# fchchen/omni-recall-rag

Measured on AMD Instinct MI355X. Metric: queries/sec at top-k=10 over N x 3072-d chunks; score delta vs C# reference in `parity`, higher is better.
Workload: dtype i8 screen + f32*f32->f64 exact re-score; 1 GPU; C3: 10000000 chunks x 3072-d fp32 on one GPU, batch=256 queries per step, top-k=10, full hybrid (cosine+keyword+recency), candidate_limit=corpus; corpus_rows=10000000

## Files before the change

### omni-recall-rag_amd/csrc/orr_epilogue.h

```cpp
#pragma once

#include "orr_kernels.h"
#include "orr_device.h"

#include <type_traits>

#include "orr_screen_tile16_asm.inc"

namespace orr {

typedef float f32x16 __attribute__((ext_vector_type(16)));
typedef __bf16 bf16x8 __attribute__((ext_vector_type(8)));
typedef __bf16 bf16x4 __attribute__((ext_vector_type(4)));
typedef int i32x16 __attribute__((ext_vector_type(16)));
typedef int i32x4e __attribute__((ext_vector_type(4)));

constexpr int kEpiQueue = 8;
struct EpiParked { float a; uint32_t idx; };

template <int NI, int NJ>
struct EpiTileLoads {
    double2 rc[NJ];
    float4 rf[NJ];
    uint32_t w[NI][NJ][kCountPlanes];
};

template <int NI, int NJ>
__device__ __forceinline__ void epilogue_issue_loads(EpiTileLoads<NI, NJ> &L, int qbase, int64_t colbase, int32_t B, int64_t n_rows,
                                                     const FusedEpilogue &epi, int lane)
{
    const int fr = lane & 31;
    const int32_t n_qg = (B + 31) >> 5;
    const bool has_rf = epi.i8_rowf != nullptr, has_cp = epi.count_planes != nullptr;
    const float4 *rowf = has_rf ? epi.i8_rowf : reinterpret_cast<const float4 *>(epi.rowc);
#pragma unroll
    for (int j = 0; j < NJ; ++j) {
        const int64_t col = colbase + j * 32 + fr;
        const uint32_t colc = (uint32_t)(col < n_rows ? col : n_rows - 1);
        L.rc[j] = load_global(epi.rowc, colc);
        const float4 rf = load_global(rowf, colc);
        L.rf[j] = has_rf ? rf : make_float4(1.f, 0.f, 0.f, 0.f);
#pragma unroll
        for (int i = 0; i < NI; ++i) {
            const int qg = (qbase + i * 32) >> 5;
            const int qgc = qg < n_qg ? qg : n_qg - 1;
#pragma unroll
            for (int p = 0; p < kCountPlanes; ++p) {
                const gptr<uint32_t> plane = as_global(has_cp ? epi.count_planes + ((int64_t)p * n_qg + qgc) * epi.plane_stride
                                                              : reinterpret_cast<const uint32_t *>(epi.rowc));
                const uint32_t wv = plane[colc];
                L.w[i][j][p] = has_cp ? wv : 0u;
            }
        }
    }
}

template <bool AGPR, typename T>
__device__ __forceinline__ float acc_as_float(T v)
{
    if constexpr (AGPR) {
        T r;
        asm("v_accvgpr_read_b32 %0, %1" : "=v"(r) : "a"(v));
        return (float)r;
    } else {
        return (float)v;
    }
}

struct EpiNoHook { __device__ __forceinline__ void operator()(int) const {} };

template <int NI, int NJ, bool RESCORED, typename ACC = f32x16, bool STAGED = false, int QDEPTH = kEpiQueue, bool AGPR = false,
          typename HOOK = EpiNoHook>
__device__ __forceinline__ void fused_epilogue(const ACC (&acc)[NI][NJ], int qbase, int64_t colbase, int32_t B,
                                               int64_t n_rows, const FusedEpilogue &epi, int lane, EpiParked *queue,
                                               int queue_stride, uint32_t idx_salt = 0, unsigned long long *st = nullptr,
                                               const EpiTileLoads<NI, NJ> *pre = nullptr, const float4 *qf_lds = nullptr,
                                               HOOK between_blocks = HOOK())
{
    constexpr bool INT_ACC = !__is_same(ACC, f32x16);
#define ORR_EPI_STAMP(k) if (st && lane == 0) st[k] = __builtin_amdgcn_s_memtime()
    const int fr = lane & 31, fh = lane >> 5;
    EpiTileLoads<NI, NJ> own;
    if constexpr (!STAGED) epilogue_issue_loads(own, qbase, colbase, B, n_rows, epi, lane);
    const EpiTileLoads<NI, NJ> &L = STAGED ? *pre : own;
    float rb[NJ], cj[NJ], eb[NJ];
    int64_t cols[NJ];
    bool ok[NJ];
#pragma unroll
    for (int j = 0; j < NJ; ++j) {
        cols[j] = colbase + j * 32 + fr;
        ok[j] = cols[j] < n_rows;
        rb[j] = (float)L.rc[j].x;
        const float rr = ok[j] ? (float)L.rc[j].y : -__builtin_huge_valf();
        float ea = 0.f;
        eb[j] = 0.f;
        if (epi.i8_rowf) {
            rb[j] *= L.rf[j].x;
            ea = L.rf[j].y; eb[j] = L.rf[j].z;
        }
        cj[j] = rr + ea;
    }
    if (st) { asm volatile("" :: "v"(cj[0]), "v"(rb[0]), "v"(eb[0])); ORR_EPI_STAMP(4); }
    int parked = 0;
    auto qf_of = [&](int i, int e) -> float4 {
        const int qi = qbase + i * 32 + (e & 3) + 8 * (e >> 2) + 4 * fh;
        if constexpr (STAGED) return qf_lds[i * 32 + (e & 3) + 8 * (e >> 2) + 4 * fh];
        else return epi.qf[qi < B ? qi : B - 1];
    };
#pragma unroll
    for (int i = 0; i < NI; ++i) {
        between_blocks(i);
        uint32_t w[NJ][kCountPlanes];
#pragma unroll
        for (int j = 0; j < NJ; ++j)
#pragma unroll
            for (int p = 0; p < kCountPlanes; ++p) w[j][p] = L.w[i][j][p] >> (16 * fh);
        const int q_left = B - (qbase + i * 32 + 4 * fh);
        if constexpr (STAGED) {
            unsigned long long wave_any = 0ull;
            float4 qfg[2][4];
#pragma unroll
            for (int e = 0; e < 4; ++e) qfg[0][e] = qf_of(i, e);
#pragma unroll
            for (int e0 = 0; e0 < 16; e0 += 4) {
                if (e0 + 4 < 16) {
#pragma unroll
                    for (int e = 0; e < 4; ++e) qfg[((e0 >> 2) + 1) & 1][e] = qf_of(i, e0 + 4 + e);
                }
                __builtin_amdgcn_sched_barrier(0);
                unsigned long long hit[4][NJ];
#pragma unroll
                for (int e1 = 0; e1 < 4; ++e1) {
                    const int e = e0 + e1;
                    const float4 qf = qfg[(e0 >> 2) & 1][e1];
#pragma unroll
                    for (int j = 0; j < NJ; ++j) {
                        const uint32_t m = (w[j][e >> 2] >> (4 * (e & 3))) & 15u;
                        const float a = acc_as_float<AGPR>(acc[i][j][e]);
                        const float upper = __builtin_fmaf((float)m, qf.z, __builtin_fmaf(a, qf.x * rb[j], __builtin_fmaf(qf.w, eb[j], cj[j])));
                        hit[e1][j] = __builtin_amdgcn_ballot_w64(!(upper < qf.y));
                    }
                }
#pragma unroll
                for (int e1 = 0; e1 < 4; ++e1)
#pragma unroll
                    for (int j = 0; j < NJ; ++j) wave_any |= hit[e1][j];
            }
            if (wave_any == 0ull) {
                if (i == 0) { ORR_EPI_STAMP(5); }
                continue;
            }
        }
#pragma unroll
        for (int e = 0; e < 16; ++e) {
            const int cb = (e & 3) + 8 * (e >> 2);
            const int qi = qbase + i * 32 + cb + 4 * fh;
            const float4 qf = qf_of(i, e);
            const bool has_query = cb < q_left;
#pragma unroll
            for (int j = 0; j < NJ; ++j) {
                const uint32_t m = (w[j][e >> 2] >> (4 * (e & 3))) & 15u;
                const float a = acc_as_float<AGPR>(acc[i][j][e]);
                const float upper = __builtin_fmaf((float)m, qf.z, __builtin_fmaf(a, qf.x * rb[j], __builtin_fmaf(qf.w, eb[j], cj[j])));
                bool drop = upper < qf.y;
                if constexpr (!INT_ACC) drop = drop && __builtin_fabsf(a) <= 3.4028234663852886e38f;
                drop = drop || !has_query || !ok[j];
                if (!drop) {
                    if (parked < QDEPTH) {
                        EpiParked pk;
                        pk.a = a; pk.idx = (uint32_t)((i * 16 + e) * NJ + j) + idx_salt;
                        queue[parked * queue_stride] = pk;
                    } else if (RESCORED) {
                        const uint32_t slot = atomicAdd(&epi.cnt[qi], 1u);
                        if (slot < epi.cap) {
                            SelEntry en;
                            en.key = ~0ull; en.pos = (uint32_t)cols[j]; en.pad = 0;
                            epi.buf[(int64_t)qi * epi.cap + slot] = en;
                        }
                    } else {
                        atomicAdd(&epi.cnt[qi], epi.cap + 1u);
                    }
                    ++parked;
                }
            }
        }
        if (i == 0) { ORR_EPI_STAMP(5); }
    }
    ORR_EPI_STAMP(6);
#undef ORR_EPI_STAMP
    if (parked > QDEPTH) parked = QDEPTH;
    for (int s = 0; s < parked; ++s) {
        EpiParked pk = queue[s * queue_stride];
        pk.idx -= idx_salt;
        const int j = (int)(pk.idx % NJ), ie = (int)(pk.idx / NJ), e = ie & 15, i = ie >> 4;
        const int qi = qbase + i * 32 + (e & 3) + 8 * (e >> 2) + 4 * fh;
        const int64_t col = colbase + j * 32 + fr;
        const QueryConst qc = epi.qc[qi];
        const double2 rc = epi.rowc[col];
        const uint32_t mm = qc.n_terms > 0 ? kw_matches(epi.kw, qi, (uint32_t)col) : 0u;
        double dot = (double)pk.a, bound = 0.0;
        if (epi.i8_rowf) {
            const float4 rf = epi.i8_rowf[col];
            dot *= (double)rf.x * (double)epi.i8_qs1[qi];
            bound = (double)rf.y + (double)epi.qf[qi].w * (double)rf.z;
        }
        unsigned long long key = score_key(fused_score_fast(dot, rc.x, rc.y, mm, qc) + bound);
        if (!(__builtin_fabsf(pk.a) <= 3.4028234663852886e38f) || !(bound <= 1.7976931348623157e308)) key = ~0ull;
        if (key > epi.tau[qi]) {
            const uint32_t slot = atomicAdd(&epi.cnt[qi], 1u);
            if (slot < epi.cap) {
                SelEntry en;
                en.key = key; en.pos = (uint32_t)col; en.pad = 0;
                epi.buf[(int64_t)qi * epi.cap + slot] = en;
            }
        }
    }
}

__device__ __forceinline__ int tile16_row(int m) { return (((0 - (m >> 2)) & 3) << 2) | (m & 3); }
__device__ __forceinline__ int tile16_c_of(int lane) { return tile16_row(lane & 15); }
__device__ __forceinline__ int tile16_g_of(int lane) { return (0 - (lane >> 4)) & 3; }

struct EpiTileLoads16 {
    double2 rc[8];
    float4 rf[8];
    uint32_t w[4][8][2];
};

template <int BITS = 4>
__device__ __forceinline__ void epilogue_word_offsets16(uint32_t (&at)[8], int64_t colbase, int32_t B, int64_t n_rows, const FusedEpilogue &epi,
                                                        int lane)
{
    const int c = tile16_c_of(lane), g = tile16_g_of(lane);
    const int32_t n_qg = (B + 31) >> 5;
    const uint32_t plane_dist = epi.count_planes && BITS == 4 ? (uint32_t)((int64_t)n_qg * epi.plane_stride) : 0u;
    const uint32_t col0 = (uint32_t)colbase + (uint32_t)c, last = (uint32_t)(n_rows - 1), half = (uint32_t)(g >> 1) * plane_dist;
#pragma unroll
    for (int j = 0; j < 8; ++j) {
        const uint32_t col = col0 + 16u * j;
        at[j] = (col < last ? col : last) + half;
    }
}

template <int BITS = 4>
__device__ __forceinline__ void epilogue_load_words16(uint32_t (&w)[8][2], const uint32_t (&at)[8], int b, int qbase, int32_t B,
                                                      const FusedEpilogue &epi)
{
    const int32_t n_qg = (B + 31) >> 5;
    const bool has_cp = epi.count_planes != nullptr;
    const int qg = (qbase >> 5) + b;
    const int qgc = qg < n_qg ? qg : n_qg - 1;
#pragma unroll
    for (int t = 0; t < 2; ++t) {
        const uint32_t *plane = has_cp ? epi.count_planes + ((int64_t)(BITS == 2 ? t : 2 * t) * n_qg + qgc) * epi.plane_stride
                                       : reinterpret_cast<const uint32_t *>(epi.rowc);
#pragma unroll
        for (int j = 0; j < 8; ++j) {
            const uint32_t wv = load_global_at<uint32_t>(plane, at[j] * 4u);
            w[j][t] = has_cp ? wv : 0u;
        }
    }
}

template <int BITS = 4>
__device__ __forceinline__ void epilogue_issue_loads16(EpiTileLoads16 &L, int qbase, int64_t colbase, int32_t B, int64_t n_rows,
                                                       const FusedEpilogue &epi, int lane)
{
    const uint32_t col0 = (uint32_t)colbase + (uint32_t)tile16_c_of(lane), last = (uint32_t)(n_rows - 1);
#pragma unroll
    for (int j = 0; j < 8; ++j) {
        const uint32_t col = col0 + 16u * j;
        const uint32_t off = (col < last ? col : last) * 16u;
        L.rc[j] = load_global_at_d2(epi.rowc, off);
        L.rf[j] = load_global_at_f4(epi.i8_rowf, off);
    }
    uint32_t at[8];
    epilogue_word_offsets16<BITS>(at, colbase, B, n_rows, epi, lane);
    epilogue_load_words16<BITS>(L.w[0], at, 0, qbase, B, epi);
}

template <int BITS = 4>
__device__ __forceinline__ void epilogue_issue_later_words16(EpiTileLoads16 &L, int qbase, int64_t colbase, int32_t B, int64_t n_rows,
                                                             const FusedEpilogue &epi, int lane)
{
    uint32_t at[8];
    epilogue_word_offsets16<BITS>(at, colbase, B, n_rows, epi, lane);
#pragma unroll
    for (int b = 1; b < 4; ++b) epilogue_load_words16<BITS>(L.w[b], at, b, qbase, B, epi);
}

template <int N, typename F>
__device__ __forceinline__ void static_for(F &&f)
{
    if constexpr (N > 0) {
        static_for<N - 1>(f);
        f(std::integral_constant<int, N - 1>{});
    }
}

template <int IDX>
__device__ __forceinline__ float acc16_as_float(int token)
{
    int r;
    asm("v_accvgpr_read_b32 %0, a[%1]" : "=v"(r) : "n"(IDX), "v"(token) : ORR_T16_ACC_CLOBBERS);
    return (float)r;
}

template <int IDX>
__device__ __forceinline__ float acc16_as_float_here(int token)
{
    int r;
    asm volatile("v_accvgpr_read_b32 %0, a[%1]" : "=v"(r) : "n"(IDX), "v"(token) : ORR_T16_ACC_CLOBBERS);
    return (float)r;
}

template <int IDX>
__device__ __forceinline__ int acc16_as_int_here(int token)
{
    int r;
    asm volatile("v_accvgpr_read_b32 %0, a[%1]" : "=v"(r) : "n"(IDX), "v"(token) : ORR_T16_ACC_CLOBBERS);
    return r;
}

typedef float f32x2e __attribute__((ext_vector_type(2)));

__host__ __device__ constexpr uint32_t count_nibbles_even(uint32_t w) { return w & 0x0F0F0F0Fu; }
__host__ __device__ constexpr uint32_t count_nibbles_odd(uint32_t w) { return (w >> 4) & 0x0F0F0F0Fu; }
__host__ __device__ constexpr uint32_t count_nibble_operand(int e, uint32_t x, uint32_t y) { return (e & 1) ? y : x; }
__host__ __device__ constexpr int count_nibble_byte(int e) { return e >> 1; }

__host__ __device__ constexpr uint32_t spread_count_fields2(uint32_t v)
{
    const uint32_t t = v | (v << 6);
    return (t | (t << 12)) & 0x03030303u;
}

namespace count_word_checks {
constexpr bool two_bit_spread_exact()
{
    for (uint32_t v = 0; v < 256u; ++v)
        for (int e = 0; e < 4; ++e)
            if (((spread_count_fields2(v) >> (8 * e)) & 0xFFu) != ((v >> (2 * e)) & 3u)) return false;
    return true;
}
constexpr bool nibble_extraction_exact()
{
    for (int h = 0; h < 2; ++h)
        for (int e = 0; e < 4; ++e)
            for (uint32_t v = 0; v < 16u; ++v)
                for (uint32_t bg : {0u, ~0u}) {
                    const int at = 16 * h + 4 * e;
                    const uint32_t w = (bg & ~(15u << at)) | (v << at);
                    const uint32_t half = w >> (16 * h);
                    const uint32_t op = count_nibble_operand(e, count_nibbles_even(half), count_nibbles_odd(half));
                    if (((op >> (8 * count_nibble_byte(e))) & 0xFFu) != v) return false;
                }
    return true;
}
}
static_assert(count_word_checks::two_bit_spread_exact(), "two-bit count words: field e of a byte must land in byte e");
static_assert(count_word_checks::nibble_extraction_exact(), "four-bit count words: nibble e must be byte (e >> 1) of x or y");

template <int E>
__device__ __forceinline__ float count_of_nibble(uint32_t x, uint32_t y)
{
    const uint32_t v = count_nibble_operand(E, x, y);
    float r;
    if constexpr (count_nibble_byte(E) == 0) asm("v_cvt_f32_ubyte0 %0, %1" : "=v"(r) : "v"(v));
    else asm("v_cvt_f32_ubyte1 %0, %1" : "=v"(r) : "v"(v));
    return r;
}

template <int BYTE>
__device__ __forceinline__ float ubyte_as_float(uint32_t v)
{
    float r;
    if constexpr (BYTE == 0) asm("v_cvt_f32_ubyte0 %0, %1" : "=v"(r) : "v"(v));
    else if constexpr (BYTE == 1) asm("v_cvt_f32_ubyte1 %0, %1" : "=v"(r) : "v"(v));
    else if constexpr (BYTE == 2) asm("v_cvt_f32_ubyte2 %0, %1" : "=v"(r) : "v"(v));
    else asm("v_cvt_f32_ubyte3 %0, %1" : "=v"(r) : "v"(v));
    return r;
}

template <int QDEPTH, typename HOOK = EpiNoHook, int BITS = 4>
__device__ __forceinline__ void fused_epilogue16(int acc_token, int qbase, int64_t colbase, int32_t B, int64_t n_rows,
                                                 const FusedEpilogue &epi, int lane, EpiParked *queue, int queue_stride, uint32_t idx_salt,
                                                 unsigned long long *st, const EpiTileLoads16 &L, const float4 *qf_lds,
                                                 HOOK between_blocks = HOOK())
{
#define ORR_EPI_STAMP(k) if (st && lane == 0) st[k] = __builtin_amdgcn_s_memtime()
    const int c = tile16_c_of(lane), g = tile16_g_of(lane);
    const int sh = 16 * (g & 1);
    const float qw_max = qf_lds[0].w;
    f32x2e rb2[4], cjw2[4];
    const int64_t col0 = colbase + c;
#pragma unroll
    for (int j = 0; j < 8; ++j) {
        const float rbv = (float)L.rc[j].x * L.rf[j].x;
        const float cj = (float)L.rc[j].y + L.rf[j].y, eb = L.rf[j].z;
        const bool keep_all = !(rbv <= 1e30f) || !(eb <= 1e30f) || !(cj <= 3.0e38f) || !(cj >= -3.0e38f);
        const float cjw = keep_all ? __builtin_huge_valf() : __builtin_fmaf(qw_max, eb, cj);
        rb2[j >> 1][j & 1] = keep_all ? 0.f : rbv;
        cjw2[j >> 1][j & 1] = col0 + j * 16 < n_rows ? cjw : -__builtin_huge_valf();
    }
    if (st) { asm volatile("" :: "v"(cjw2[0][0]), "v"(rb2[0][0])); ORR_EPI_STAMP(4); }
    int parked = 0;
    const float4 *qf_lane = qf_lds + 4 * g;
    uint32_t group_flags = 0u;
    static_for<4>([&](auto b_c) {
        constexpr int b = decltype(b_c)::value;
        between_blocks(b);
        static_for<2>([&](auto t_c) {
            constexpr int t = decltype(t_c)::value;
            f32x2e qx2[4], qz2[4], nqy2[4];
            float mx[4];
#pragma unroll
            for (int e = 0; e < 4; ++e) {
                const float4 qf = qf_lane[32 * b + 16 * t + e];
                qx2[e] = f32x2e{qf.x, qf.x}; qz2[e] = f32x2e{qf.z, qf.z}; nqy2[e] = f32x2e{-qf.y, -qf.y};
                mx[e] = -__builtin_huge_valf();
            }
            static_for<4>([&](auto jp_c) {
                constexpr int jp = decltype(jp_c)::value, j0 = 2 * jp;
                uint32_t x0, y0, x1, y1;
                if constexpr (BITS == 2) {
                    x0 = spread_count_fields2(__builtin_amdgcn_ubfe(L.w[b][j0][t], 8u * (uint32_t)g, 8u));
                    x1 = spread_count_fields2(__builtin_amdgcn_ubfe(L.w[b][j0 + 1][t], 8u * (uint32_t)g, 8u));
                    y0 = y1 = 0u;
                } else {
                    const uint32_t w0 = L.w[b][j0][t] >> sh, w1 = L.w[b][j0 + 1][t] >> sh;
                    x0 = count_nibbles_even(w0); y0 = count_nibbles_odd(w0); x1 = count_nibbles_even(w1); y1 = count_nibbles_odd(w1);
                }
                static_for<4>([&](auto e_c) {
                    constexpr int e = decltype(e_c)::value;
                    const f32x2e a2 = {acc16_as_float<4 * (8 * (2 * b + t) + j0) + e>(acc_token), acc16_as_float<4 * (8 * (2 * b + t) + j0 + 1) + e>(acc_token)};
                    f32x2e m2;
                    if constexpr (BITS == 2) m2 = f32x2e{ubyte_as_float<e>(x0), ubyte_as_float<e>(x1)};
                    else m2 = f32x2e{count_of_nibble<e>(x0, y0), count_of_nibble<e>(x1, y1)};
                    const f32x2e t1 = a2 * rb2[jp];
                    const f32x2e t2 = __builtin_elementwise_fma(t1, qx2[e], cjw2[jp]);
                    const f32x2e t3 = __builtin_elementwise_fma(m2, qz2[e], t2);
                    const f32x2e d = t3 + nqy2[e];
                    mx[e] = __builtin_fmaxf(__builtin_fmaxf(mx[e], d[0]), d[1]);
                });
            });
#pragma unroll
            for (int e = 0; e < 4; ++e) {
                const unsigned long long group_any = __builtin_amdgcn_ballot_w64(mx[e] >= 0.f);
                group_flags |= group_any != 0ull ? 1u << (8 * b + 4 * t + e) : 0u;
            }
            asm volatile("" :: "s"(group_flags));
        });
        if constexpr (b == 0) { ORR_EPI_STAMP(5); }
    });
    int token_1b = acc_token;
    asm volatile("" : "+v"(token_1b));
    static_for<4>([&](auto b_c) {
        constexpr int b = decltype(b_c)::value;
        if (((group_flags >> (8 * b)) & 0xffu) != 0u) {
            uint32_t at1[8], w1[8][2];
            epilogue_word_offsets16<BITS>(at1, colbase, B, n_rows, epi, lane);
            epilogue_load_words16<BITS>(w1, at1, b, qbase, B, epi);
            static_for<8>([&](auto te_c) {
                constexpr int te = decltype(te_c)::value, t = te >> 2, e = te & 3, i = 2 * b + t;
                if ((group_flags & (1u << (8 * b + te))) == 0u) return;
                const int qi = qbase + 16 * i + 4 * g + e;
                const float4 q1 = qf_lane[32 * b + 16 * t + e];
                const bool has_query = qi < B;
                static_for<8>([&](auto j_c) {
                    constexpr int j = decltype(j_c)::value;
                    const uint32_t m = BITS == 2 ? (w1[j][t] >> (8 * g + 2 * e)) & 3u : ((w1[j][t] >> sh) >> (4 * e)) & 15u;
                    const float a = acc16_as_float_here<4 * (8 * i + j) + e>(token_1b);
                    const float upper = __builtin_fmaf((float)m, q1.z, __builtin_fmaf(a * rb2[j >> 1][j & 1], q1.x, cjw2[j >> 1][j & 1]));
                    const bool drop = upper < q1.y || !has_query || !(col0 + j * 16 < n_rows);
                    if (!drop) {
                        if (parked < QDEPTH) {
                            EpiParked pk;
                            pk.a = a; pk.idx = (uint32_t)((i * 4 + e) * 8 + j) + idx_salt;
                            queue[parked * queue_stride] = pk;
                        } else {
                            const uint32_t slot = atomicAdd(&epi.cnt[qi], 1u);
                            if (slot < epi.cap) {
                                SelEntry en;
                                en.key = ~0ull; en.pos = (uint32_t)(col0 + j * 16); en.pad = 0;
                                epi.buf[(int64_t)qi * epi.cap + slot] = en;
                            }
                        }
                        ++parked;
                    }
                });
            });
        }
    });
    ORR_EPI_STAMP(6);
#undef ORR_EPI_STAMP
    if (parked > QDEPTH) parked = QDEPTH;
    for (int s = 0; s < parked; ++s) {
        EpiParked pk = queue[s * queue_stride];
        pk.idx -= idx_salt;
        const int j = (int)(pk.idx & 7u), ie = (int)(pk.idx >> 3), e = ie & 3, i = ie >> 2;
        const int qi = qbase + 16 * i + 4 * g + e;
        const int64_t col = colbase + j * 16 + c;
        const QueryConst qc = epi.qc[qi];
        const double2 rc = epi.rowc[col];
        const uint32_t mm = qc.n_terms > 0 ? kw_matches(epi.kw, qi, (uint32_t)col) : 0u;
        const float4 rf = epi.i8_rowf[col];
        const double dot = (double)pk.a * ((double)rf.x * (double)epi.i8_qs1[qi]);
        const double bound = (double)rf.y + (double)epi.qf[qi].w * (double)rf.z;
        unsigned long long key = score_key(fused_score_fast(dot, rc.x, rc.y, mm, qc) + bound);
        if (!(bound <= 1.7976931348623157e308)) key = ~0ull;
        if (key > epi.tau[qi]) {
            const uint32_t slot = atomicAdd(&epi.cnt[qi], 1u);
            if (slot < epi.cap) {
                SelEntry en;
                en.key = key; en.pos = (uint32_t)col; en.pad = 0;
                epi.buf[(int64_t)qi * epi.cap + slot] = en;
            }
        }
    }
}

}
```

Before: 31390 queries/s.

## Add coarse per-lane bound gate before per-column screen bound evaluation

Replaces the per-column float bound computation in the screening epilogue with a two-level gate. First, each lane takes the max integer accumulator over its 8 columns, combined with the max row scale, the max offset and an OR/max-combined keyword count field, to form a cheap upper bound per query group. Only groups whose coarse bound passes run the finer per-column float bound, which now uses the group-wide count bound instead of per-column counts. This cuts VALU work and count-field unpacking in the common all-rejected case. In exchange, the finer pass is looser on the count term, so slightly more groups may reach the exact stage, and it adds a second accumulator-read pass for the groups that pass.

```diff
diff --git a/omni-recall-rag_amd/csrc/orr_epilogue.h b/omni-recall-rag_amd/csrc/orr_epilogue.h
--- a/omni-recall-rag_amd/csrc/orr_epilogue.h
+++ b/omni-recall-rag_amd/csrc/orr_epilogue.h
@@ -307,6 +307,14 @@
 }
 
 template <int IDX>
+__device__ __forceinline__ int acc16_as_int(int token)
+{
+    int r;
+    asm("v_accvgpr_read_b32 %0, a[%1]" : "=v"(r) : "n"(IDX), "v"(token) : ORR_T16_ACC_CLOBBERS);
+    return r;
+}
+
+template <int IDX>
 __device__ __forceinline__ float acc16_as_float_here(int token)
 {
     int r;
@@ -324,63 +332,50 @@
 
 typedef float f32x2e __attribute__((ext_vector_type(2)));
 
-__host__ __device__ constexpr uint32_t count_nibbles_even(uint32_t w) { return w & 0x0F0F0F0Fu; }
-__host__ __device__ constexpr uint32_t count_nibbles_odd(uint32_t w) { return (w >> 4) & 0x0F0F0F0Fu; }
-__host__ __device__ constexpr uint32_t count_nibble_operand(int e, uint32_t x, uint32_t y) { return (e & 1) ? y : x; }
-__host__ __device__ constexpr int count_nibble_byte(int e) { return e >> 1; }
-
-__host__ __device__ constexpr uint32_t spread_count_fields2(uint32_t v)
-{
-    const uint32_t t = v | (v << 6);
-    return (t | (t << 12)) & 0x03030303u;
-}
+template <int BITS, int N>
+__host__ __device__ constexpr uint32_t count_group_bound(const uint32_t (&w)[N])
+{
+    uint32_t any = 0u, three = 0u;
+    for (int j = 0; j < N; ++j) {
+        any |= w[j];
+        if (BITS == 2) three |= w[j] & (w[j] >> 1);
+    }
+    return BITS == 2 ? any & ~(any & (any >> 1) & ~three & 0x55555555u) : any;
+}
+template <int BITS>
+__host__ __device__ constexpr uint32_t count_lane_fields(uint32_t w, int g) { return BITS == 2 ? w >> (8 * g) : w >> (16 * (g & 1)); }
+template <int BITS>
+__host__ __device__ constexpr uint32_t count_field_of(uint32_t lane_fields, int e) { return (lane_fields >> (BITS * e)) & ((1u << BITS) - 1u); }
 
 namespace count_word_checks {
-constexpr bool two_bit_spread_exact()
-{
-    for (uint32_t v = 0; v < 256u; ++v)
-        for (int e = 0; e < 4; ++e)
-            if (((spread_count_fields2(v) >> (8 * e)) & 0xFFu) != ((v >> (2 * e)) & 3u)) return false;
+template <int BITS, int ROWS>
+constexpr bool group_bound_covers_every_row()
+{
+    constexpr uint32_t top = (1u << BITS) - 1u;
+    uint32_t combos = 1u;
+    for (int r = 0; r < ROWS; ++r) combos *= top + 1u;
+    for (int g = 0; g < 4; ++g)
+        for (int e = 0; e < 4; ++e) {
+            const int at = BITS == 2 ? 8 * g + 2 * e : 16 * (g & 1) + 4 * e;
+            for (uint32_t c = 0; c < combos; ++c)
+                for (uint32_t bg : {0u, ~0u}) {
+                    uint32_t w[ROWS] = {}, largest = 0u, ored = 0u;
+                    for (uint32_t r = 0, rest = c; r < (uint32_t)ROWS; ++r, rest >>= BITS) {
+                        const uint32_t v = rest & top;
+                        w[r] = ((r & 1u ? ~bg : bg) & ~(top << at)) | (v << at);
+                        largest = v > largest ? v : largest;
+                        ored |= v;
+                        if (count_field_of<BITS>(count_lane_fields<BITS>(w[r], g), e) != v) return false;
+                    }
+                    const uint32_t got = count_field_of<BITS>(count_lane_fields<BITS>(count_group_bound<BITS>(w), g), e);
+                    if (BITS == 2 ? got != largest : (got != ored || got < largest)) return false;
+                }
+        }
     return true;
 }
-constexpr bool nibble_extraction_exact()
-{
-    for (int h = 0; h < 2; ++h)
-        for (int e = 0; e < 4; ++e)
-            for (uint32_t v = 0; v < 16u; ++v)
-                for (uint32_t bg : {0u, ~0u}) {
-                    const int at = 16 * h + 4 * e;
-                    const uint32_t w = (bg & ~(15u << at)) | (v << at);
-                    const uint32_t half = w >> (16 * h);
-                    const uint32_t op = count_nibble_operand(e, count_nibbles_even(half), count_nibbles_odd(half));
-                    if (((op >> (8 * count_nibble_byte(e))) & 0xFFu) != v) return false;
-                }
-    return true;
-}
-}
-static_assert(count_word_checks::two_bit_spread_exact(), "two-bit count words: field e of a byte must land in byte e");
-static_assert(count_word_checks::nibble_extraction_exact(), "four-bit count words: nibble e must be byte (e >> 1) of x or y");
-
-template <int E>
-__device__ __forceinline__ float count_of_nibble(uint32_t x, uint32_t y)
-{
-    const uint32_t v = count_nibble_operand(E, x, y);
-    float r;
-    if constexpr (count_nibble_byte(E) == 0) asm("v_cvt_f32_ubyte0 %0, %1" : "=v"(r) : "v"(v));
-    else asm("v_cvt_f32_ubyte1 %0, %1" : "=v"(r) : "v"(v));
-    return r;
-}
-
-template <int BYTE>
-__device__ __forceinline__ float ubyte_as_float(uint32_t v)
-{
-    float r;
-    if constexpr (BYTE == 0) asm("v_cvt_f32_ubyte0 %0, %1" : "=v"(r) : "v"(v));
-    else if constexpr (BYTE == 1) asm("v_cvt_f32_ubyte1 %0, %1" : "=v"(r) : "v"(v));
-    else if constexpr (BYTE == 2) asm("v_cvt_f32_ubyte2 %0, %1" : "=v"(r) : "v"(v));
-    else asm("v_cvt_f32_ubyte3 %0, %1" : "=v"(r) : "v"(v));
-    return r;
-}
+}
+static_assert(count_word_checks::group_bound_covers_every_row<2, 3>(), "two-bit count words: a field of the group's word must be the largest of the rows' fields");
+static_assert(count_word_checks::group_bound_covers_every_row<4, 2>(), "four-bit count words: a field of the group's word must be >= that field of every row");
 
 template <int QDEPTH, typename HOOK = EpiNoHook, int BITS = 4>
 __device__ __forceinline__ void fused_epilogue16(int acc_token, int qbase, int64_t colbase, int32_t B, int64_t n_rows,
@@ -398,63 +393,74 @@
     for (int j = 0; j < 8; ++j) {
         const float rbv = (float)L.rc[j].x * L.rf[j].x;
         const float cj = (float)L.rc[j].y + L.rf[j].y, eb = L.rf[j].z;
-        const bool keep_all = !(rbv <= 1e30f) || !(eb <= 1e30f) || !(cj <= 3.0e38f) || !(cj >= -3.0e38f);
+        const bool keep_all = !(rbv >= 0.f) || !(rbv <= 1e30f) || !(eb <= 1e30f) || !(cj <= 3.0e38f) || !(cj >= -3.0e38f);
         const float cjw = keep_all ? __builtin_huge_valf() : __builtin_fmaf(qw_max, eb, cj);
         rb2[j >> 1][j & 1] = keep_all ? 0.f : rbv;
         cjw2[j >> 1][j & 1] = col0 + j * 16 < n_rows ? cjw : -__builtin_huge_valf();
     }
     if (st) { asm volatile("" :: "v"(cjw2[0][0]), "v"(rb2[0][0])); ORR_EPI_STAMP(4); }
+    const float rb_max = __builtin_fmaxf(__builtin_fmaxf(__builtin_fmaxf(rb2[0][0], rb2[0][1]), __builtin_fmaxf(rb2[1][0], rb2[1][1])),
+                                         __builtin_fmaxf(__builtin_fmaxf(rb2[2][0], rb2[2][1]), __builtin_fmaxf(rb2[3][0], rb2[3][1])));
+    const float cjw_max = __builtin_fmaxf(__builtin_fmaxf(__builtin_fmaxf(cjw2[0][0], cjw2[0][1]), __builtin_fmaxf(cjw2[1][0], cjw2[1][1])),
+                                          __builtin_fmaxf(__builtin_fmaxf(cjw2[2][0], cjw2[2][1]), __builtin_fmaxf(cjw2[3][0], cjw2[3][1])));
     int parked = 0;
     const float4 *qf_lane = qf_lds + 4 * g;
-    uint32_t group_flags = 0u;
+    uint32_t gate_open = 0u, lane_fields[4][2];
     static_for<4>([&](auto b_c) {
         constexpr int b = decltype(b_c)::value;
         between_blocks(b);
         static_for<2>([&](auto t_c) {
             constexpr int t = decltype(t_c)::value;
-            f32x2e qx2[4], qz2[4], nqy2[4];
-            float mx[4];
-#pragma unroll
-            for (int e = 0; e < 4; ++e) {
+            const uint32_t wrows[8] = {L.w[b][0][t], L.w[b][1][t], L.w[b][2][t], L.w[b][3][t], L.w[b][4][t], L.w[b][5][t], L.w[b][6][t], L.w[b][7][t]};
+            const uint32_t wmine = count_lane_fields<BITS>(count_group_bound<BITS>(wrows), g);
+            lane_fields[b][t] = wmine;
+            static_for<4>([&](auto e_c) {
+                constexpr int e = decltype(e_c)::value;
                 const float4 qf = qf_lane[32 * b + 16 * t + e];
-                qx2[e] = f32x2e{qf.x, qf.x}; qz2[e] = f32x2e{qf.z, qf.z}; nqy2[e] = f32x2e{-qf.y, -qf.y};
-                mx[e] = -__builtin_huge_valf();
-            }
-            static_for<4>([&](auto jp_c) {
-                constexpr int jp = decltype(jp_c)::value, j0 = 2 * jp;
-                uint32_t x0, y0, x1, y1;
-                if constexpr (BITS == 2) {
-                    x0 = spread_count_fields2(__builtin_amdgcn_ubfe(L.w[b][j0][t], 8u * (uint32_t)g, 8u));
-                    x1 = spread_count_fields2(__builtin_amdgcn_ubfe(L.w[b][j0 + 1][t], 8u * (uint32_t)g, 8u));
-                    y0 = y1 = 0u;
-                } else {
-                    const uint32_t w0 = L.w[b][j0][t] >> sh, w1 = L.w[b][j0 + 1][t] >> sh;
-                    x0 = count_nibbles_even(w0); y0 = count_nibbles_odd(w0); x1 = count_nibbles_even(w1); y1 = count_nibbles_odd(w1);
-                }
-                static_for<4>([&](auto e_c) {
-                    constexpr int e = decltype(e_c)::value;
-                    const f32x2e a2 = {acc16_as_float<4 * (8 * (2 * b + t) + j0) + e>(acc_token), acc16_as_float<4 * (8 * (2 * b + t) + j0 + 1) + e>(acc_token)};
-                    f32x2e m2;
-                    if constexpr (BITS == 2) m2 = f32x2e{ubyte_as_float<e>(x0), ubyte_as_float<e>(x1)};
-                    else m2 = f32x2e{count_of_nibble<e>(x0, y0), count_of_nibble<e>(x1, y1)};
-                    const f32x2e t1 = a2 * rb2[jp];
-                    const f32x2e t2 = __builtin_elementwise_fma(t1, qx2[e], cjw2[jp]);
-                    const f32x2e t3 = __builtin_elementwise_fma(m2, qz2[e], t2);
-                    const f32x2e d = t3 + nqy2[e];
-                    mx[e] = __builtin_fmaxf(__builtin_fmaxf(mx[e], d[0]), d[1]);
+                int a_max = 0;
+                static_for<4>([&](auto jp_c) {
+                    constexpr int j0 = 2 * decltype(jp_c)::value;
+                    const int a0 = acc16_as_int<4 * (8 * (2 * b + t) + j0) + e>(acc_token), a1 = acc16_as_int<4 * (8 * (2 * b + t) + j0 + 1) + e>(acc_token);
+                    a_max = a_max > a0 ? a_max : a0;
+                    a_max = a_max > a1 ? a_max : a1;
                 });
+                const float m_max = (float)count_field_of<BITS>(wmine, e);
+                const float cos_max = __builtin_fmaf((float)a_max * rb_max, qf.x, cjw_max);
+                const float d = __builtin_fmaf(m_max, qf.z, cos_max) - qf.y;
+                const unsigned long long group_any = __builtin_amdgcn_ballot_w64(d >= 0.f);
+                gate_open |= group_any != 0ull ? 1u << (8 * b + 4 * t + e) : 0u;
             });
-#pragma unroll
-            for (int e = 0; e < 4; ++e) {
-                const unsigned long long group_any = __builtin_amdgcn_ballot_w64(mx[e] >= 0.f);
-                group_flags |= group_any != 0ull ? 1u << (8 * b + 4 * t + e) : 0u;
-            }
-            asm volatile("" :: "s"(group_flags));
+            asm volatile("" :: "s"(gate_open));
         });
         if constexpr (b == 0) { ORR_EPI_STAMP(5); }
     });
+    uint32_t group_flags = 0u;
+    asm volatile("" : "+s"(gate_open));
+    if (gate_open != 0u) {
+        int token_1a = acc_token;
+        asm volatile("" : "+v"(token_1a));
+        static_for<32>([&](auto bte_c) {
+            constexpr int bte = decltype(bte_c)::value, b = bte >> 3, t = (bte >> 2) & 1, e = bte & 3;
+            if ((gate_open & (1u << bte)) == 0u) return;
+            const float4 qf = qf_lane[32 * b + 16 * t + e];
+            const f32x2e qx2 = {qf.x, qf.x};
+            float mx = -__builtin_huge_valf();
+            static_for<4>([&](auto jp_c) {
+                constexpr int jp = decltype(jp_c)::value, j0 = 2 * jp;
+                const f32x2e a2 = {acc16_as_float_here<4 * (8 * (2 * b + t) + j0) + e>(token_1a), acc16_as_float_here<4 * (8 * (2 * b + t) + j0 + 1) + e>(token_1a)};
+                const f32x2e t1 = a2 * rb2[jp];
+                const f32x2e t2 = __builtin_elementwise_fma(t1, qx2, cjw2[jp]);
+                mx = __builtin_fmaxf(__builtin_fmaxf(mx, t2[0]), t2[1]);
+            });
+            const float m_max = (float)count_field_of<BITS>(lane_fields[b][t], e);
+            const float d = __builtin_fmaf(m_max, qf.z, mx) - qf.y;
+            const unsigned long long group_any = __builtin_amdgcn_ballot_w64(d >= 0.f);
+            group_flags |= group_any != 0ull ? 1u << bte : 0u;
+        });
+    }
     int token_1b = acc_token;
     asm volatile("" : "+v"(token_1b));
+    asm volatile("" : "+s"(group_flags));
     static_for<4>([&](auto b_c) {
         constexpr int b = decltype(b_c)::value;
         if (((group_flags >> (8 * b)) & 0xffu) != 0u) {
```

Result: faster. 32090 queries/s, median of 6 (+2.2%).
